# kevin-robb/live_ekf_slam

Measured on AMD Instinct MI355X. Metric: EKF predict-update steps/sec @ L=50, batch=65536; fp64 state RMSE vs ref, higher is better.
Workload: dtype f64

## Files before the change

### live_ekf_slam_amd/csrc/ekf_kernel_impl.h

```cpp
#pragma once
#include "ekf_kernel.h"

#include <stdio.h>

#include <type_traits>

#include "../../include/slam_batch.h"
#include "ekf_model.h"
#include "slam_rng.h"
#include "sim_device.h"

namespace slam {

template <int NMAX, int W, int KG_, int UNR_, int KP_ = 0>
struct EkfGeom {
    static constexpr int TPB = 64 * W;
    static constexpr int LDP = (NMAX + 2) & ~1;
    static constexpr int LMAX = (NMAX - 3) / 2;
    static constexpr int KCAP = LMAX > 0 ? LMAX : 1;
    static constexpr int KG = KG_;
    static constexpr int KP = KP_ > 0 ? KP_ : ((KG_ > 5 && NMAX > 43 && W < 5) ? 3 : (KG_ > 4 ? 4 : KG_));
    static constexpr int KLOOP = 2 * KP;
    static constexpr int TS = 3 + 2 * KP;
    static constexpr int UNR = UNR_;
};

template <int VEC>
constexpr int hp_substride(int ldp) {
    int hs = (ldp + VEC - 1) / VEC;
    while ((hs % 16) != (16 / VEC) && (hs % 16) != 16 - (16 / VEC)) ++hs;
    return hs;
}

#ifdef SLAM_ABLATE
#define SLAM_DBG(x) (x)
#else
#define SLAM_DBG(x) 0
#endif

#ifndef SLAM_SLEEP_RING
#define SLAM_SLEEP_RING 1
#endif
#ifndef SLAM_SLEEP_LEADER
#define SLAM_SLEEP_LEADER 2
#endif
#ifndef SLAM_SLEEP_PASS
#define SLAM_SLEEP_PASS 1
#endif
#ifndef SLAM_PASS_MIN
#define SLAM_PASS_MIN 4
#endif
#ifndef SLAM_W1_WAVES
#define SLAM_W1_WAVES 3
#endif
#ifndef SLAM_SD
#define SLAM_SD 3
#endif
#ifndef SLAM_CTRL_ILP
#define SLAM_CTRL_ILP 1
#endif
#ifndef SLAM_CTRL_SG
#define SLAM_CTRL_SG 3
#endif
#ifndef SLAM_PRIO_THIN
#define SLAM_PRIO_THIN 2
#endif

#define SLAM_STAMP(i)                                                                    \
    do {                                                                                 \
        if (prof_on && tid == 0) {                                                       \
            const unsigned long long now_ = __builtin_readcyclecounter();                \
            p.prof[(size_t)blockIdx.x * kEkfProfSlots + (i)] += now_ - tprev;                            \
            tprev = now_;                                                                \
        }                                                                                \
    } while (0)

typedef double dbl2_t __attribute__((ext_vector_type(2)));
typedef float flt4_t __attribute__((ext_vector_type(4)));
template <class ST> struct Vec16;
template <> struct Vec16<double> {
    static constexpr int VEC = 2;
    typedef dbl2_t type;
};
template <> struct Vec16<float> {
    static constexpr int VEC = 4;
    typedef flt4_t type;
};

__device__ __forceinline__ int opaque(int v) {
    asm volatile("" : "+v"(v));
    return v;
}

typedef const __attribute__((address_space(4))) EkfStepParams* EkfColdParams;
__device__ __forceinline__ EkfColdParams ekf_cold_params() {
    EkfColdParams k = (EkfColdParams)__builtin_amdgcn_kernarg_segment_ptr();
    asm volatile("" : "+s"(k));
    return k;
}
struct EkfSimCold {
    uint64_t seed;
    int64_t inst0;
    double d_max, th_max, range_max, fov_min, fov_max;
};
struct EkfMapCold {
    const double* map;
    const double* map_each;
    const int32_t* L_each;
    int32_t map_stride, L;
};
struct EkfSimNoiseCold {
    double sV00, sV11, sW00, sW11;
    const NoiseRow* noise_each;
    int32_t sim;
};

__device__ __forceinline__ double rdlane(double v, int l) {
    const int lo = __builtin_amdgcn_readlane(__double2loint(v), l);
    const int hi = __builtin_amdgcn_readlane(__double2hiint(v), l);
    return __hiloint2double(hi, lo);
}

__device__ __forceinline__ unsigned hi_abs(double v) {
    return (unsigned)(__double_as_longlong(v) >> 32) & 0x7fffffffu;
}

template <int NMAX, int W, int KG_, int UNR_, class ST, int PIPE, bool MULTI, int KP_ = 0>
__global__ __launch_bounds__(64 * W, (W >= 2 ? 4 : SLAM_W1_WAVES)) void ekf_step_kernel(const EkfStepParams p) {
    using G = EkfGeom<NMAX, W, KG_, UNR_, KP_>;
    constexpr int TPB = G::TPB, LDP = G::LDP, KCAP = G::KCAP, LMAX = G::LMAX, KG = G::KG, KP = G::KP, KLOOP = G::KLOOP, TS = G::TS, UNR = G::UNR;

    __shared__ double s_xt[LDP];
    __shared__ double s_xp[LDP];
    __shared__ double s_R[TS * LDP];
    __shared__ double s_C[TS * LDP];
    __shared__ double2 s_K[KG * LDP];
    constexpr int VEC = Vec16<ST>::VEC;
    constexpr int HS = hp_substride<VEC>(LDP), HPW = (VEC - 1) * HS + (LDP + VEC - 1) / VEC;
    __shared__ double2 s_HP[KG * HPW];
    __shared__ double s_sc[16];
    constexpr int SD = SLAM_SD;
    __shared__ float s_meas[SD * 3 * KCAP];
    __shared__ double s_tru[SD * 6];
    __shared__ int s_kraw[SD];
    __shared__ int s_sim[2];
    __shared__ int s_ids[LMAX > 0 ? LMAX : 1];
    __shared__ int s_didx[2 * KCAP];
    __shared__ int s_next[2 * 4];
    __shared__ double s_ps[2 * 10];
    __shared__ int s_chunk;
    __shared__ int s_T[TS];
    __shared__ signed char s_slot[LDP];
    __shared__ signed char s_need[TS];
    __shared__ int s_misc[8];
    __shared__ double s_keep[4];
    __shared__ int s_kh[8];
    __shared__ int s_ring[8];
    __shared__ int s_pass[4];
    __shared__ int s_wend[KG];
    __shared__ unsigned s_cnt[4];

    const int b = blockIdx.x;
    const int tid = threadIdx.x;
    const int lane = tid & 63;
    const FilterNoise nz = filter_noise(p, b);
    if (p.long_mode == 1) {
        const int kk = p.meas_count_in[b];
        if ((kk < p.k_stride_in ? kk : p.k_stride_in) > p.long_cap) return;
    }

    const bool dump_meas = p.meas_out != nullptr;
    const bool prof_on = (p.dbg & 4) && p.prof != nullptr;
    unsigned long long tprev = prof_on ? __builtin_readcyclecounter() : 0ull;
    if (prof_on && tid < 64) p.prof[(size_t)blockIdx.x * kEkfProfSlots + tid] = 0ull;
    typedef typename Vec16<ST>::type VT;
    constexpr int ESZ = (int)sizeof(ST);
    auto hpi = [](int c) -> int { return (c & (VEC - 1)) * HS + (c / VEC); };
    const int T = MULTI ? p.T : 1;
    ST* const PA = const_cast<ST*>(static_cast<const ST*>(p.P)) + (size_t)b * p.pstride;
    ST* const PB = static_cast<ST*>(p.P_out) + (size_t)b * p.pstride;
    ST* const Pfinal = PA;
    ST* Pcur = PA;
    ST* __restrict__ xb = static_cast<ST*>(p.x) + (size_t)b * p.xstride;
    constexpr bool kWide = sizeof(ST) == 8;
    int flags = p.flags[b];
    const int M_init = p.M[b];
    double xpre[(LDP + TPB - 1) / TPB];
#pragma unroll
    for (int u = 0; u < (LDP + TPB - 1) / TPB; ++u) {
        const int i = tid + TPB * u;
        xpre[u] = (i < p.xstride && i < LDP) ? (double)xb[i] : 0.0;
    }
    const int idpre = (tid < p.L_max) ? p.ids[(size_t)b * p.L_max + tid] : 0;
    double keep0 = 0.0;
    if (p.sim && tid < 64) {
        if (tid < 3) keep0 = p.truth[3 * (size_t)b + tid];
        if (tid == 3) keep0 = p.err_sum[b];
    }
    const int n_init = 3 + 2 * M_init;
    const int ts0 = p.timestep[b];

    if (flags & SLAM_INST_INDEX_OOR) {
        return;
    }

#pragma unroll
    for (int u = 0; u < (LDP + TPB - 1) / TPB; ++u) {
        const int i = tid + TPB * u;
        if (i < LDP) {
            const double v = i < n_init ? xpre[u] : 0.0;
            s_xt[i] = v;
            s_xp[i] = v;
        }
    }
    if (tid < M_init) s_ids[tid] = idpre;
    if (tid < 4) s_keep[tid] = keep0;
#pragma unroll 1
    for (int i = tid; i < LDP; i += TPB) s_slot[i] = (signed char)(i < 3 ? i : -1);
    if (tid < TS) {
        s_T[tid] = tid < 3 ? tid : -1;
        s_need[tid] = (signed char)(tid < 3 ? 1 : 0);
    }
    if (tid < 8) s_kh[tid] = 0;
    if (tid < KG) s_wend[tid] = 0;
    if (tid < 2) s_sim[tid] = 0;
    if (tid < 4) s_cnt[tid] = tid == 1 ? (unsigned)((n_init + M_init / 2 + 8) * ESZ / 8) : 0u;
    auto count_pass = [](unsigned* cnt, int vec16, int nupd) {
        atomicAdd(&cnt[0], (unsigned)vec16);
        atomicAdd(&cnt[2], 1u);
        atomicAdd(&cnt[3], (unsigned)nupd);
    };
    auto count_other = [](unsigned* cnt, int elems) { atomicAdd(&cnt[1], (unsigned)(elems * ESZ) / 8u); };

#include "ekf_step_prestep.h"
#include "ekf_step_control.h"
#include "ekf_step_stream.h"
    if (W == 1) pregather(tid, TPB);
    else if (tid >= 64) pregather(tid - 64, TPB - 64);
    if (tid == TPB - 1) count_other(s_cnt, 6 * n_init);
    if (tid < 64) prestep(0);
    if (tid >= TPB - 3) s_need[tid - (TPB - 3)] = 0;
    SLAM_STAMP(1);

    bool wd_fired = false;
    int frz_at = -1, frz_M = 0, frz_n = 0;
    const ST* frz_P = nullptr;
#pragma unroll 1
    for (int t = 0; t < T; ++t) {
    const ST* const Pin = Pcur;
    const int pb = t & 1;
    const float* const meas_t = s_meas + (t % SD) * 3 * KCAP;
    int* const didx_t = s_didx + pb * KCAP;
    const int M_old = M;
    const int n_old = na;
    if (tid < 8) s_misc[tid] = 0;
    __builtin_amdgcn_s_setprio(SLAM_PRIO_THIN);
    __syncthreads();
    const int kraw = s_next[4 * pb];
    if (kraw > KCAP) flags |= SLAM_INST_CAPACITY;
    const int k = kraw < KCAP ? kraw : KCAP;
    if (tid == 0) s_kh[k < 7 ? k : 7] += 1;
    if (p.sim && dump_meas && t == T - 1) {
        const EkfColdParams pc = ekf_cold_params();
        const int kso = pc->k_stride_out;
        float* const mo = pc->meas_out + (size_t)b * kso * 3;
        for (int i = tid; i < 3 * k && i < 3 * kso; i += TPB) mo[i] = meas_t[i];
        if (tid == 0) pc->meas_count_out[b] = k;
    }
    const int room_ins = (p.L_max < LMAX ? p.L_max : LMAX) - M_old;
    const int n_ins = p.id_known ? s_next[4 * pb + 1] : (k < room_ins ? k : (room_ins > 0 ? room_ins : 0));
    const bool frz_top = p.id_known && s_next[4 * pb + 2];
    if (p.id_known && s_next[4 * pb + 3]) flags |= SLAM_INST_CAPACITY;
    SLAM_STAMP(2);

#include "ekf_step_decoupled.h"
#include "ekf_step_lockstep.h"
    const int te = opaque(tid);
    for (int i = te; i < na; i += TPB) {
        const ST sv = (ST)s_xp[i];
        s_xt[i] = (double)sv;
        s_xp[i] = (double)sv;
        const unsigned h0 = hi_abs((double)sv);
        hiacc = hiacc > h0 ? hiacc : h0;
    }
    if constexpr (!kWide) {
        if (t + 1 < T) {
            const int nTl = s_misc[5];
#pragma unroll 1
            for (int i = te; i < nTl * LDP; i += TPB) {
                s_R[i] = (double)(ST)s_R[i];
                s_C[i] = (double)(ST)s_C[i];
            }
        }
    }
    if (s_misc[6]) flags |= SLAM_INST_S_SINGULAR;
    const bool nonfinite = __syncthreads_or(hiacc >= 0x7ff00000u);
    if (nonfinite) flags |= SLAM_INST_NONFINITE;

    if (na != nf) {
        const int ldf = ekf_ld(nf, ESZ), lda = ekf_ld(na, ESZ);
        if (tid == 0) count_other(s_cnt, 2 * na * na);
#pragma unroll 1
        for (int r = 0; r < na; ++r) {
            ST tmp[(LDP + TPB - 1) / TPB];
#pragma unroll
            for (int u = 0; u < (LDP + TPB - 1) / TPB; ++u) {
                const int c = te + TPB * u;
                tmp[u] = c < na ? Pout[(size_t)r * ldf + c] : (ST)0;
            }
            __syncthreads();
#pragma unroll
            for (int u = 0; u < (LDP + TPB - 1) / TPB; ++u) {
                const int c = te + TPB * u;
                if (c < lda) Pout[(size_t)r * lda + c] = tmp[u];
            }
            __syncthreads();
        }
    }
    if ((p.dbg & 32) && p.prof != nullptr && tid == 0 && t < kEkfProfSlots)
        p.prof[(size_t)blockIdx.x * kEkfProfSlots + t] = (wall_clock64() << 4) | (unsigned long long)(k < 15 ? k : 15);
    Pcur = Pout;
    SLAM_STAMP(10);
    }

    if (wd_fired) {
        finish(0, M, flags | SLAM_INST_WATCHDOG | SLAM_INST_INDEX_OOR, true);
        return;
    }
    if (frz_at >= 0) {
        __syncthreads();
        if (Pfinal != frz_P) {
            const int nn = frz_n * ekf_ld(frz_n, ESZ);
            if (tid == 0) count_other(s_cnt, 2 * nn);
            for (int i = tid; i < nn; i += TPB) Pfinal[i] = frz_P[i];
            __syncthreads();
        }
        finish(frz_at, frz_M, flags | SLAM_INST_INDEX_OOR, true);
        return;
    }
    if (Pcur != Pfinal) {
        __syncthreads();
        const int nn = na * ekf_ld(na, ESZ);
        if (tid == 0) count_other(s_cnt, 2 * nn);
        for (int i = tid; i < nn; i += TPB) Pfinal[i] = Pcur[i];
        __syncthreads();
    }

    finish(T, M, flags, false);
    SLAM_STAMP(8);
}

template <int NMAX, int W, int KG_, int UNR_, class ST, int PIPE, int KP_>
hipError_t launch_variant(const EkfStepParams& p, hipStream_t stream) {
    if (ekf_device_cmds(p) && p.T > 1)
        hipLaunchKernelGGL((ekf_step_kernel<NMAX, W, KG_, UNR_, ST, PIPE, true, KP_>), dim3(p.B), dim3(64 * W), 0, stream, p);
    else
        hipLaunchKernelGGL((ekf_step_kernel<NMAX, W, KG_, UNR_, ST, PIPE, false, KP_>), dim3(p.B), dim3(64 * W), 0, stream, p);
    return hipGetLastError();
}

template <int NMAX, int W, int KG_, int UNR_, class ST, int PIPE, int KP_>
hipError_t variant_info(int multi, EkfKernelInfo* out) {
    const void* fn = multi ? reinterpret_cast<const void*>(&ekf_step_kernel<NMAX, W, KG_, UNR_, ST, PIPE, true, KP_>)
                           : reinterpret_cast<const void*>(&ekf_step_kernel<NMAX, W, KG_, UNR_, ST, PIPE, false, KP_>);
    hipFuncAttributes a;
    hipError_t e = hipFuncGetAttributes(&a, fn);
    if (e != hipSuccess) return e;
    int nb = 0;
    e = hipOccupancyMaxActiveBlocksPerMultiprocessor(&nb, fn, 64 * W, 0);
    if (e != hipSuccess) return e;
    snprintf(out->name, sizeof(out->name), "ekf_step_kernel<%d,%d,%d,%d,%s,%d,%s,%d>", NMAX, W, KG_, UNR_,
             sizeof(ST) == 8 ? "double" : "float", PIPE, multi ? "true" : "false", KP_);
    out->lds_bytes = (int)a.sharedSizeBytes;
    out->vgprs = a.numRegs;
    out->sgprs = 0;
    out->threads = 64 * W;
    out->wg_per_cu = nb;
    return hipSuccess;
}

}
```

### live_ekf_slam_amd/csrc/ekf_step_control.h

```cpp

    auto leader_chain = [&](int ii, int si, float r_m, float b_m, double (&H)[8], double& nu0, double& nu1, double (&Si)[4]) -> bool {
        const double* const xl = p.lm_from_pred ? s_xp : s_xt;
        const double dx = xl[ii] - s_xp[0], dy = xl[ii + 1] - s_xp[1];
        const float dist = (float)sqrt(dx * dx + dy * dy);
        const double dd = (double)dist, d2 = (double)(dist * dist);
        const int hl = lane & 7;
        const bool usey = (hl == 1) || (hl == 3) || (hl == 4) || (hl == 6);
        const bool neg = (hl == 0) || (hl == 1) || (hl == 5) || (hl == 6);
        double num = usey ? dy : dx;
        num = neg ? -num : num;
        const double q = num / (hl < 4 ? dd : d2);
        const float angf = (float)rem2pi(det_atan2(dy, dx) - s_xp[2]);
        const float nu0f = r_m - dist - nz.w_r;
        const float nu1f = b_m - angf - nz.w_b;
        nu0 = (double)nu0f; nu1 = (double)nu1f;
#pragma unroll
        for (int j = 0; j < 8; ++j) H[j] = rdlane(q, j);
        const double h00 = H[0], h01 = H[1], h03 = H[2], h04 = H[3], h10 = H[4], h11 = H[5], h12 = -1.0, h13 = H[6], h14 = H[7];
        const int cs = lane < 3 ? lane : (lane == 3 ? ii : ii + 1);
        const double p0 = s_R[cs], p1 = s_R[LDP + cs], p2 = s_R[2 * LDP + cs], pi = s_R[si * LDP + cs], pj = s_R[(si + 1) * LDP + cs];
        const double gx = ((h00 * p0 + h01 * p1) + h03 * pi) + h04 * pj;
        const double gy = (((h10 * p0 + h11 * p1) + h12 * p2) + h13 * pi) + h14 * pj;
        const double g0x = rdlane(gx, 0), g1x = rdlane(gx, 1), g2x = rdlane(gx, 2), gix = rdlane(gx, 3), gjx = rdlane(gx, 4);
        const double g0y = rdlane(gy, 0), g1y = rdlane(gy, 1), g2y = rdlane(gy, 2), giy = rdlane(gy, 3), gjy = rdlane(gy, 4);
        double S[4];
        S[0] = ((g0x * h00 + g1x * h01) + gix * h03) + gjx * h04;
        S[1] = (((g0x * h10 + g1x * h11) + g2x * h12) + gix * h13) + gjx * h14;
        S[2] = ((g0y * h00 + g1y * h01) + giy * h03) + gjy * h04;
        S[3] = (((g0y * h10 + g1y * h11) + g2y * h12) + giy * h13) + gjy * h14;
        S[0] = S[0] + nz.W00;
        S[3] = S[3] + nz.W11;
        return inv2x2_lu(S, Si);
    };

    auto form_known = [&](const int* didx_g, int k, int l0, int lim, int nsrc, int& l1_out, int& nT_out) -> int {
        const int l1 = (k - l0 < lim) ? k : l0 + lim;
        const int ng = l1 - l0;
        const int idx = (lane < ng) ? didx_g[l0 + lane] : -1;
        const int myii = idx >= 0 ? 3 + 2 * idx : -1;
        const int cur = (lane < KP) ? s_T[3 + 2 * lane] : -1;
        bool dupl = false, has = false, keep = false;
#pragma unroll
        for (int w = 0; w < KP; ++w) {
            const int ii_w = __builtin_amdgcn_readlane(myii, w), cur_w = __builtin_amdgcn_readlane(cur, w);
            dupl = dupl || (w < lane && ii_w == myii);
            has = has || (cur_w >= 0 && cur_w == myii);
            keep = keep || (ii_w >= 0 && ii_w == cur);
        }
        const bool wantv = myii >= 0 && !dupl;
        const bool release = lane < KP && cur >= 0 && !keep;
        if (release) {
            s_slot[cur] = (signed char)-1; s_slot[cur + 1] = (signed char)-1;
            s_T[3 + 2 * lane] = -1; s_T[4 + 2 * lane] = -1;
        }
        const bool freeslot = lane < KP && (cur < 0 || !keep);
        const unsigned long long fmask = __ballot(freeslot);
        const bool needs = wantv && !has;
        const unsigned long long nmask = __ballot(needs);
        const int rank = __popcll(nmask & ((1ull << lane) - 1ull));
        int j = 0;
        {
            unsigned long long fm = fmask;
#pragma unroll
            for (int w = 0; w < KP; ++w) {
                const int lowest = __ffsll((long long)fm) - 1;
                if (w == rank) j = lowest;
                fm &= fm - 1ull;
            }
        }
        bool gath = false;
        if (needs) {
            s_T[3 + 2 * j] = myii; s_T[4 + 2 * j] = myii + 1;
            s_slot[myii] = (signed char)(3 + 2 * j); s_slot[myii + 1] = (signed char)(4 + 2 * j);
            const signed char nd = (signed char)(myii < nsrc ? 1 : 2);
            s_need[3 + 2 * j] = nd; s_need[4 + 2 * j] = nd;
            gath = nd == 1;
        }
        unsigned long long occ = __ballot(lane < KP && cur >= 0 && keep);
        {
            unsigned long long fm = fmask;
            const int ntake = __popcll(nmask);
#pragma unroll
            for (int w = 0; w < KP; ++w) {
                const int lowest = __ffsll((long long)fm) - 1;
                if (w < ntake && lowest >= 0) occ |= 1ull << lowest;
                fm &= fm - 1ull;
            }
        }
        l1_out = l1;
        nT_out = occ ? 5 + 2 * (63 - __clzll((long long)occ)) : 3;
        return __ballot(gath) != 0ull ? 1 : 0;
    };

    auto thin_downdate = [&](int j0, int jstride, int s0, int sstride, int nTd, int nd, const double2* __restrict__ Ku,
                             const double2* __restrict__ HPu) {
        const int* const Ttab = s_T;
#pragma unroll 1
        for (int j = j0; j < nd; j += jstride) {
            const double2 kj = Ku[j], hj = HPu[hpi(j)];
#pragma unroll 2
            for (int sl = s0; sl < nTd; sl += sstride) {
                const int t_s = Ttab[sl];
                if ((unsigned)t_s < (unsigned)nd) {
                    const double2 kt = Ku[t_s], ht = HPu[hpi(t_s)];
                    const int i = sl * LDP + j;
                    s_R[i] = ekf_downdate(s_R[i], kt.x, kt.y, hj.x, hj.y);
                    s_C[i] = ekf_downdate(s_C[i], kj.x, kj.y, ht.x, ht.y);
                }
            }
        }
    };

    constexpr int NU = (LDP + 63) / 64;
    auto thin_downdate_ctl = [&](int nTd, int nd, const double2* __restrict__ Ku, const double2* __restrict__ HPu, const double2 (&kj)[NU],
                                 const double2 (&hj)[NU]) {
        constexpr int SG = SLAM_CTRL_SG;
        int tsv[TS];
#pragma unroll
        for (int sl = 0; sl < TS; ++sl) tsv[sl] = s_T[sl];
#pragma unroll
        for (int s0 = 0; s0 < TS; s0 += SG) {
            if (s0 >= nTd) break;
            double2 kt[SG], ht[SG];
            double rv[SG][NU], cv[SG][NU];
            bool ok[SG];
#pragma unroll
            for (int g = 0; g < SG; ++g) {
                const int sl = s0 + g < TS ? s0 + g : TS - 1;
                const int t_s = tsv[sl];
                ok[g] = s0 + g < nTd && (unsigned)t_s < (unsigned)nd;
                const int tc = ok[g] ? t_s : 0;
                kt[g] = Ku[tc]; ht[g] = HPu[hpi(tc)];
#pragma unroll
                for (int u = 0; u < NU; ++u) {
                    const int j = lane + 64 * u;
                    const int i = sl * LDP + (j < LDP ? j : 0);
                    rv[g][u] = s_R[i]; cv[g][u] = s_C[i];
                }
            }
#pragma unroll
            for (int g = 0; g < SG; ++g) {
                if (!ok[g]) continue;
                const int sl = s0 + g;
#pragma unroll
                for (int u = 0; u < NU; ++u) {
                    const int j = lane + 64 * u;
                    if (j < nd) {
                        const int i = sl * LDP + j;
                        s_R[i] = ekf_downdate(rv[g][u], kt[g].x, kt[g].y, hj[u].x, hj[u].y);
                        s_C[i] = ekf_downdate(cv[g][u], kj[u].x, kj[u].y, ht[g].x, ht[g].y);
                    }
                }
            }
        }
    };
```

### live_ekf_slam_amd/csrc/ekf_step_decoupled.h

```cpp

    if constexpr (MULTI && W >= 2) {
        auto fastable = [&](int tq) -> bool {
            const int* nx = s_next + 4 * (tq & 1);
            constexpr int kStepMax = sizeof(ST) == 8 ? KLOOP : (KLOOP < KG ? KLOOP : KG);
            return nx[0] <= kStepMax && nx[1] == 0 && nx[2] == 0 && nx[3] == 0;
        };
        const bool fast_ok = p.id_known && !dump_meas && fastable(t) &&
                             !SLAM_DBG(p.dbg & (2 | 16 | 64));
        if (fast_ok) {
            const int n = na, ldn = ekf_ld(n, ESZ);
            ST* const Pbuf = Pcur;
            constexpr int kFirstStreamer = 1;
            constexpr int NS = W - kFirstStreamer;
            constexpr bool kGen = W >= 2;
            if (tid == 0) {
                s_ring[0] = nu; s_ring[1] = 0; s_ring[2] = 0; s_ring[3] = 0; s_ring[4] = t; s_ring[5] = 0; s_ring[6] = 0; s_ring[7] = 0;
                s_pass[0] = 0; s_pass[1] = 0; s_pass[2] = 0; s_pass[3] = 0;
            }
            __syncthreads();
            auto ld_i = [](int* q) -> int { return __hip_atomic_load(q, __ATOMIC_RELAXED, __HIP_MEMORY_SCOPE_WORKGROUP); };
            auto st_i = [](int* q, int v) { __hip_atomic_store(q, v, __ATOMIC_RELAXED, __HIP_MEMORY_SCOPE_WORKGROUP); };
            constexpr int kSpinBudget = 1 << 21;
            auto spin_over = [&](int& spins) -> bool {
                spins += 1;
                if (spins > kSpinBudget) st_i(&s_ring[2], 1);
                return ld_i(&s_ring[2]) != 0;
            };

            bool is_streamer = true;
            if (tid < 64) {
                is_streamer = false;
                __builtin_amdgcn_s_setprio(3);
                int tt = t;
                int pub = nu;
                int fl_or = 0;
                bool first_it = true;
#pragma unroll 1
                for (;;) {
                    const int pq = tt & 1;
                    const float* const meas_q = s_meas + (tt % SD) * 3 * KCAP;
                    const int* const didx_q = s_didx + pq * KCAP;
                    const int kq = s_next[4 * pq];
                    if (lane == 0) st_i(&s_sim[1], tt);
                    if (!first_it && lane == 0) s_kh[kq < 7 ? kq : 7] += 1;
                    first_it = false;
                    if (lane < 3) s_xp[lane] = s_ps[10 * pq + lane];
                    SLAM_STAMP(16);
                    int lastu = -1;
                    if constexpr (!kWide) {
                        const bool isupd = lane < kq && didx_q[lane] >= 0;
                        const unsigned long long um = __ballot(isupd);
                        lastu = um ? 63 - __clzll((long long)um) : -1;
                    }
                    int l0q = 0, l1q, nTq;
#pragma unroll 1
                    do {
                    const int needg = form_known(didx_q, kq, l0q, KP, n, l1q, nTq);
                    SLAM_STAMP(17);
                    const bool veh = s_need[0] == 1;
                    if (needg || veh) {
                        if (lane == 0) st_i(&s_ring[6], 1);
                        __builtin_amdgcn_fence(__ATOMIC_SEQ_CST, "workgroup");
                        for (int sp = 0; ld_i(&s_ring[7]) && !spin_over(sp);) __builtin_amdgcn_s_sleep(1);
                        __builtin_amdgcn_fence(__ATOMIC_ACQUIRE, "workgroup");
                        const int app = ld_i(&s_ring[1]);
                        int sl = 0;
#pragma unroll 1
                        while (sl < nTq) {
                            constexpr int GB = 2;
                            int ss[GB], ts[GB], nb = 0;
#pragma unroll
                            for (int g = 0; g < GB; ++g) { ss[g] = 0; ts[g] = 0; }
#pragma unroll 1
                            while (sl < nTq && nb < GB) {
                                if (s_need[sl] == 1) {
#pragma unroll
                                    for (int g = 0; g < GB; ++g)
                                        if (g == nb) { ss[g] = sl; ts[g] = s_T[sl]; }
                                    nb += 1;
                                }
                                sl += 1;
                            }
                            if (nb == 0) break;
                            if (lane == 0) count_other(s_cnt, 2 * nb * n);
#pragma unroll 1
                            for (int j = lane; j < LDP; j += 64) {
                                double rv[GB], cv[GB];
                                const int jc = j < n ? j : 0;
#pragma unroll
                                for (int g = 0; g < GB; ++g) {
                                    rv[g] = (double)Pbuf[(size_t)ts[g] * ldn + jc];
                                    cv[g] = (double)Pbuf[(size_t)jc * ldn + ts[g]];
                                }
#pragma unroll 1
                                for (int u = app; u < pub; ++u) {
                                    const int us = u % KG;
                                    const double2* Ku = s_K + us * LDP;
                                    const double2* HPu = s_HP + us * HPW;
                                    const double2 kj = Ku[jc], hj = HPu[hpi(jc)];
                                    bool we = false;
                                    if constexpr (!kWide) we = s_wend[us] != 0;
#pragma unroll
                                    for (int g = 0; g < GB; ++g) {
                                        const double2 kt = Ku[ts[g]], ht = HPu[hpi(ts[g])];
                                        rv[g] = ekf_downdate(rv[g], kt.x, kt.y, hj.x, hj.y);
                                        cv[g] = ekf_downdate(cv[g], kj.x, kj.y, ht.x, ht.y);
                                        if constexpr (!kWide) {
                                            if (we) { rv[g] = (double)(ST)rv[g]; cv[g] = (double)(ST)cv[g]; }
                                        }
                                    }
                                }
#pragma unroll
                                for (int g = 0; g < GB; ++g)
                                    if (g < nb) {
                                        s_R[ss[g] * LDP + j] = j < n ? rv[g] : 0.0;
                                        s_C[ss[g] * LDP + j] = j < n ? cv[g] : 0.0;
                                    }
                            }
#pragma unroll
                            for (int g = 0; g < GB; ++g)
                                if (g < nb && ss[g] >= 3 && lane < 3) {
                                    s_R[ss[g] * LDP + lane] = s_C[lane * LDP + ts[g]];
                                    s_C[ss[g] * LDP + lane] = s_R[lane * LDP + ts[g]];
                                }
                        }
                        if (lane == 0) st_i(&s_ring[6], 0);
                    }
                    if (lane < TS) s_need[lane] = 0;
                    SLAM_STAMP(18);
                    if (l0q == 0) {
                        const double* const ps = s_ps + 10 * pq;
                        const double* const r2o = s_R + 2 * LDP;
                        const double* const c2o = s_C + 2 * LDP;
                        const double fa = ps[3], fb = ps[4];
                        const double p22 = r2o[2];
                        auto predicted = [&](double tv, int r, int cc) -> double {
                            const double f_r = r == 0 ? fa : fb;
                            if (r < 2) tv = tv + f_r * r2o[cc];
                            if (cc < 2) {
                                double a2 = c2o[r];
                                if (r < 2) a2 = a2 + f_r * p22;
                                tv = tv + a2 * (cc == 0 ? fa : fb);
                            }
                            if (r < 2 && cc < 2) tv = tv + ps[5 + 2 * r + cc];
                            if (r == 2 && cc == 2) tv = tv + nz.V11;
                            return tv;
                        };
                        double n_r0 = 0.0, n_r1 = 0.0, n_c0 = 0.0, n_c1 = 0.0, n_22 = 0.0;
                        const int t_s = (lane >= 2 && lane < nTq) ? s_T[lane] : -1;
                        const bool thin_l = (unsigned)t_s < (unsigned)n;
                        if (thin_l) {
                            n_r0 = predicted(s_R[lane * LDP + 0], t_s, 0);
                            n_r1 = predicted(s_R[lane * LDP + 1], t_s, 1);
                            n_c0 = predicted(s_C[lane * LDP + 0], 0, t_s);
                            n_c1 = predicted(s_C[lane * LDP + 1], 1, t_s);
                            if (lane == 2) n_22 = predicted(p22, 2, 2);
                        }
#pragma unroll
                        for (int u = 0; u < (LDP + 63) / 64; ++u) {
                            const int j = lane + 64 * u;
                            if (j >= 2 && j < n) {
                                const double r2 = r2o[j], c2 = c2o[j];
                                s_R[j] = ekf_pred_row(s_R[j], fa, r2);
                                s_R[LDP + j] = ekf_pred_row(s_R[LDP + j], fb, r2);
                                s_C[j] = ekf_pred_col(s_C[j], c2, fa);
                                s_C[LDP + j] = ekf_pred_col(s_C[LDP + j], c2, fb);
                            }
                        }
                        if (lane < 2) {
                            const int j = lane;
                            const double v00 = predicted(s_R[j], 0, j), v10 = predicted(s_R[LDP + j], 1, j);
                            const double w00 = predicted(s_C[j], j, 0), w10 = predicted(s_C[LDP + j], j, 1);
                            s_R[j] = v00; s_R[LDP + j] = v10; s_C[j] = w00; s_C[LDP + j] = w10;
                        }
                        if (thin_l) {
                            s_R[lane * LDP + 0] = n_r0; s_R[lane * LDP + 1] = n_r1;
                            s_C[lane * LDP + 0] = n_c0; s_C[lane * LDP + 1] = n_c1;
                            if (lane == 2) { s_R[2 * LDP + 2] = n_22; s_C[2 * LDP + 2] = n_22; }
                        }
                    }
                    SLAM_STAMP(19);
#pragma unroll 1
                    for (int l = l0q; l < l1q; ++l) {
                        const int idx = didx_q[l];
                        if (idx < 0) continue;
                        const float r_m = meas_q[3 * l + 1], b_m = meas_q[3 * l + 2];
                        const int ii = 3 + 2 * idx;
                        const int si = s_slot[ii];
                        double H[8], Si[4], nu0, nu1;
                        if (!leader_chain(ii, si, r_m, b_m, H, nu0, nu1, Si)) fl_or |= SLAM_INST_S_SINGULAR;
                        SLAM_STAMP(20);
                        for (int sp = 0; pub - ld_i(&s_ring[1]) >= KG && !spin_over(sp);) __builtin_amdgcn_s_sleep(SLAM_SLEEP_RING);
                        if (ld_i(&s_ring[2])) break;
                        SLAM_STAMP(21);
                        const int slot = pub % KG;
                        double2* __restrict__ HPu = s_HP + slot * HPW;
                        double2* __restrict__ Ku = s_K + slot * LDP;
                        double2 kreg[NU], hreg[NU];
#pragma unroll
                        for (int u = 0; u < NU; ++u) { kreg[u] = make_double2(0.0, 0.0); hreg[u] = make_double2(0.0, 0.0); }
                        if (!SLAM_DBG(p.dbg & 512)) {
                            const double h00 = H[0], h01 = H[1], h03 = H[2], h04 = H[3], h10 = H[4], h11 = H[5], h12 = -1.0, h13 = H[6], h14 = H[7];
                            const double* Ri = s_R + si * LDP;
                            const double* Rj = s_R + (si + 1) * LDP;
                            const double* Ci = s_C + si * LDP;
                            const double* Cj = s_C + (si + 1) * LDP;
#pragma unroll
                            for (int u = 0; u < (LDP + 63) / 64; ++u) {
                                const int c = lane + 64 * u;
                                double2 hp = make_double2(0.0, 0.0), kk = make_double2(0.0, 0.0);
                                if (c < n) {
                                    const double p0 = s_R[c], p1 = s_R[LDP + c], p2 = s_R[2 * LDP + c], pi = Ri[c], pj = Rj[c];
                                    hp.x = ((h00 * p0 + h01 * p1) + h03 * pi) + h04 * pj;
                                    hp.y = (((h10 * p0 + h11 * p1) + h12 * p2) + h13 * pi) + h14 * pj;
                                    const double q0 = s_C[c], q1 = s_C[LDP + c], q2 = s_C[2 * LDP + c], qi = Ci[c], qj = Cj[c];
                                    const double phx = ((q0 * h00 + q1 * h01) + qi * h03) + qj * h04;
                                    const double phy = (((q0 * h10 + q1 * h11) + q2 * h12) + qi * h13) + qj * h14;
                                    kk.x = phx * Si[0] + phy * Si[2];
                                    kk.y = phx * Si[1] + phy * Si[3];
                                    double xv = s_xp[c] + (kk.x * nu0 + kk.y * nu1);
                                    if (c == 2) xv = rem2pi(xv);
                                    s_xp[c] = xv;
                                }
                                if (c < LDP) { HPu[hpi(c)] = hp; Ku[c] = kk; }
                                kreg[u] = kk; hreg[u] = hp;
                            }
                        }
                        if (!kWide && lane == 0) s_wend[slot] = (l == lastu) ? 1 : 0;
                        __builtin_amdgcn_fence(__ATOMIC_RELEASE, "workgroup");
                        pub += 1;
                        if (lane == 0) st_i(&s_ring[0], pub);
                        SLAM_STAMP(22);
                        if (!SLAM_DBG(p.dbg & 256)) {
#if SLAM_CTRL_ILP
                            thin_downdate_ctl(nTq, n, Ku, HPu, kreg, hreg);
#else
                            thin_downdate(lane, 64, 0, 1, nTq, n, Ku, HPu);
#endif
                        }
                    }
                    l0q = l1q;
                    } while (l0q < kq && !ld_i(&s_ring[2]));
                    if (ld_i(&s_ring[2])) break;
                    SLAM_STAMP(23);
                    if (p.sim && lane == 0) {
                        const double* tru = s_tru + (tt % SD) * 6 + 3;
                        const double ex = (double)(float)s_xp[0] - tru[0], ey = (double)(float)s_xp[1] - tru[1];
                        s_keep[3] = s_keep[3] + sqrt(ex * ex + ey * ey);
                    }
#pragma unroll 1
                    for (int i = lane; i < n; i += 64) {
                        const ST sv = (ST)s_xp[i];
                        s_xt[i] = (double)sv;
                        s_xp[i] = (double)sv;
                        const unsigned h0 = hi_abs((double)sv);
                        hiacc = hiacc > h0 ? hiacc : h0;
                    }
                    if constexpr (!kWide) {
                        const int nel = nTq * LDP;
#pragma unroll 1
                        for (int i0 = lane; i0 < nel; i0 += 256) {
                            double rv[4], cv[4];
#pragma unroll
                            for (int u = 0; u < 4; ++u) {
                                const int i = i0 + 64 * u < nel ? i0 + 64 * u : i0;
                                rv[u] = s_R[i]; cv[u] = s_C[i];
                            }
#pragma unroll
                            for (int u = 0; u < 4; ++u) {
                                const int i = i0 + 64 * u;
                                if (i < nel) { s_R[i] = (double)(ST)rv[u]; s_C[i] = (double)(ST)cv[u]; }
                            }
                        }
                    }
                    if ((p.dbg & 32) && p.prof != nullptr && lane == 0 && tt < kEkfProfSlots)
                        p.prof[(size_t)blockIdx.x * kEkfProfSlots + tt] = (wall_clock64() << 4) | (unsigned long long)(kq < 15 ? kq : 15);
                    tt += 1;
                    SLAM_STAMP(24);
                    if (tt >= T) break;
                    if constexpr (kGen) {
                        for (int sp = 0; ld_i(&s_sim[0]) <= tt && !spin_over(sp);) __builtin_amdgcn_s_sleep(1);
                        __builtin_amdgcn_fence(__ATOMIC_ACQUIRE, "workgroup");
                    }
                    SLAM_STAMP(26);
                    prestep(tt);
                    SLAM_STAMP(25);
                    if (!fastable(tt)) break;
                }
                if (lane == 0) {
                    s_ring[4] = tt;
                    s_ring[5] = fl_or;
                    __builtin_amdgcn_fence(__ATOMIC_RELEASE, "workgroup");
                    st_i(&s_ring[3], 1);
                    if (ld_i(&s_ring[2])) st_i(&s_ring[6], 0);
                }
                __builtin_amdgcn_s_setprio(0);
            }
            if (is_streamer) {
                __builtin_amdgcn_s_setprio(0);
                const bool leader = (tid >> 6) == kFirstStreamer;
#ifdef SLAM_PASS_MIN_FORCE
                constexpr int kPassMinCfg = SLAM_PASS_MIN_FORCE;
#else
#ifdef SLAM_PASS_MIN_F32
                constexpr int kPassMinF32 = SLAM_PASS_MIN_F32;
#else
                constexpr int kPassMinF32 = KG > 4 ? KG - 2 : 3;
#endif
                constexpr int kPassMinCfg = kWide ? (KG > SLAM_PASS_MIN + 1 ? KG - 1 : SLAM_PASS_MIN) : kPassMinF32;
#endif
                constexpr int kPassMin = kPassMinCfg < KG ? kPassMinCfg : KG;
                int seen = 0;
                int sp = 0;
#pragma unroll 1
                for (;;) {
                    if (leader) {
                        int app, pend;
                        bool stop = false;
#pragma unroll 1
                        for (;;) {
                            if (spin_over(sp)) { stop = true; break; }
                            app = ld_i(&s_ring[1]);
                            pend = ld_i(&s_ring[0]) - app;
                            const int ex = ld_i(&s_ring[3]);
                            if (pend > 0 && (pend >= kPassMin || ex) && !ld_i(&s_ring[6])) break;
                            if (ex && pend == 0) {
                                if (ld_i(&s_ring[0]) - app == 0) { stop = true; break; }
                                continue;
                            }
                            if constexpr (W == 2) {
                                const int ts = ld_i(&s_sim[0]);
                                if (ts < T && ts < ld_i(&s_sim[1]) + SD && !ex) {
                                    simgen(ts);
                                    __builtin_amdgcn_fence(__ATOMIC_RELEASE, "workgroup");
                                    if (lane == 0) st_i(&s_sim[0], ts + 1);
                                    continue;
                                }
                            }
                            __builtin_amdgcn_s_sleep(SLAM_SLEEP_LEADER);
                        }
                        int cnt = pend < KG ? pend : KG;
                        if constexpr (!kWide) {
                            if (!stop) {
                                while (cnt > 0 && !ld_i(&s_wend[(app + cnt - 1) % KG])) cnt -= 1;
                                if (cnt == 0) { __builtin_amdgcn_s_sleep(1); continue; }
                            }
                        }
                        if (!stop) {
                            if (lane == 0) st_i(&s_ring[7], 1);
                            __builtin_amdgcn_fence(__ATOMIC_SEQ_CST, "workgroup");
                            if (ld_i(&s_ring[6])) {
                                if (lane == 0) st_i(&s_ring[7], 0);
                                __builtin_amdgcn_s_sleep(1);
                                continue;
                            }
                        }
                        if (lane == 0) {
                            s_pass[1] = app;
                            s_pass[2] = stop ? -1 : cnt;
                            s_pass[3] = 0;
                            s_chunk = 0;
                            if (!stop) count_pass(s_cnt, 2 * n * (ldn / VEC), cnt);
                            __builtin_amdgcn_fence(__ATOMIC_RELEASE, "workgroup");
                            st_i(&s_pass[0], seen + 1);
                        }
                    }
                    while (ld_i(&s_pass[0]) <= seen && !spin_over(sp)) {
                        if constexpr (kGen && W >= 3) {
                            if ((tid >> 6) == W - 1) {
                                const int ts = ld_i(&s_sim[0]);
                                if (ts < T && ts < ld_i(&s_sim[1]) + SD && !ld_i(&s_ring[3])) {
                                    simgen(ts);
                                    __builtin_amdgcn_fence(__ATOMIC_RELEASE, "workgroup");
                                    if (lane == 0) st_i(&s_sim[0], ts + 1);
                                    continue;
                                }
                            }
                        }
                        __builtin_amdgcn_s_sleep(SLAM_SLEEP_PASS);
                    }
                    seen += 1;
                    sp = 0;
                    __builtin_amdgcn_fence(__ATOMIC_ACQUIRE, "workgroup");
                    const int lo = ld_i(&s_pass[1]), cnt = ld_i(&s_pass[2]);
                    if (cnt < 0 || ld_i(&s_ring[2])) break;
                    PassArgs pa;
                    pa.src = Pbuf; pa.dst = Pbuf; pa.mid = nullptr;
                    pa.nf = n; pa.ldd = ldn; pa.lds = ldn; pa.nsrc = n; pa.nu = cnt; pa.lo = lo;
                    stream_pass(std::integral_constant<int, 2>{}, pa);
                    __builtin_amdgcn_fence(__ATOMIC_RELEASE, "workgroup");
                    if (lane == 0) atomicAdd(&s_pass[3], 1);
                    if (leader) {
                        while (ld_i(&s_pass[3]) < NS && !spin_over(sp)) __builtin_amdgcn_s_sleep(1);
                        sp = 0;
                        if (lane == 0) {
                            if (!(p.dbg & 128)) st_i(&s_ring[1], lo + cnt);
                            st_i(&s_ring[7], 0);
                        }
                    }
                }
            }
            __syncthreads();
            if (s_ring[2]) {
                wd_fired = true;
                break;
            }
            nu = 0;
            flags |= s_ring[5];
            const int t_next = s_ring[4];
            write_vehicle(Pbuf, n);
            if (tid < KG) s_wend[tid] = 0;
            if (__syncthreads_or(hiacc >= 0x7ff00000u)) flags |= SLAM_INST_NONFINITE;
            t = t_next - 1;
            continue;
        }
    }
```

Before: 72.05 million.

## Defer ring wait past thin downdate and source tracked K/HP from registers

```diff
diff --git a/live_ekf_slam_amd/csrc/ekf_kernel_impl.h b/live_ekf_slam_amd/csrc/ekf_kernel_impl.h
--- a/live_ekf_slam_amd/csrc/ekf_kernel_impl.h
+++ b/live_ekf_slam_amd/csrc/ekf_kernel_impl.h
@@ -55,9 +55,6 @@
 #endif
 #ifndef SLAM_SD
 #define SLAM_SD 3
-#endif
-#ifndef SLAM_CTRL_ILP
-#define SLAM_CTRL_ILP 1
 #endif
 #ifndef SLAM_CTRL_SG
 #define SLAM_CTRL_SG 3
@@ -158,6 +155,7 @@
     __shared__ int s_ring[8];
     __shared__ int s_pass[4];
     __shared__ int s_wend[KG];
+    __shared__ double2 s_tKH[2 * (TS - 3)];
     __shared__ unsigned s_cnt[4];
 
     const int b = blockIdx.x;
diff --git a/live_ekf_slam_amd/csrc/ekf_step_control.h b/live_ekf_slam_amd/csrc/ekf_step_control.h
--- a/live_ekf_slam_amd/csrc/ekf_step_control.h
+++ b/live_ekf_slam_amd/csrc/ekf_step_control.h
@@ -112,8 +112,7 @@
     };
 
     constexpr int NU = (LDP + 63) / 64;
-    auto thin_downdate_ctl = [&](int nTd, int nd, const double2* __restrict__ Ku, const double2* __restrict__ HPu, const double2 (&kj)[NU],
-                                 const double2 (&hj)[NU]) {
+    auto thin_downdate_ctl = [&](int nTd, int nd, const double2 (&kj)[NU], const double2 (&hj)[NU]) {
         constexpr int SG = SLAM_CTRL_SG;
         int tsv[TS];
 #pragma unroll
@@ -129,8 +128,12 @@
                 const int sl = s0 + g < TS ? s0 + g : TS - 1;
                 const int t_s = tsv[sl];
                 ok[g] = s0 + g < nTd && (unsigned)t_s < (unsigned)nd;
-                const int tc = ok[g] ? t_s : 0;
-                kt[g] = Ku[tc]; ht[g] = HPu[hpi(tc)];
+                if (sl < 3) {
+                    kt[g] = make_double2(rdlane(kj[0].x, sl), rdlane(kj[0].y, sl));
+                    ht[g] = make_double2(rdlane(hj[0].x, sl), rdlane(hj[0].y, sl));
+                } else {
+                    kt[g] = s_tKH[2 * (sl - 3)]; ht[g] = s_tKH[2 * (sl - 3) + 1];
+                }
 #pragma unroll
                 for (int u = 0; u < NU; ++u) {
                     const int j = lane + 64 * u;
diff --git a/live_ekf_slam_amd/csrc/ekf_step_decoupled.h b/live_ekf_slam_amd/csrc/ekf_step_decoupled.h
--- a/live_ekf_slam_amd/csrc/ekf_step_decoupled.h
+++ b/live_ekf_slam_amd/csrc/ekf_step_decoupled.h
@@ -190,9 +190,8 @@
                         double H[8], Si[4], nu0, nu1;
                         if (!leader_chain(ii, si, r_m, b_m, H, nu0, nu1, Si)) fl_or |= SLAM_INST_S_SINGULAR;
                         SLAM_STAMP(20);
-                        for (int sp = 0; pub - ld_i(&s_ring[1]) >= KG && !spin_over(sp);) __builtin_amdgcn_s_sleep(SLAM_SLEEP_RING);
+                        const bool direct = pub - ld_i(&s_ring[1]) < KG;
                         if (ld_i(&s_ring[2])) break;
-                        SLAM_STAMP(21);
                         const int slot = pub % KG;
                         double2* __restrict__ HPu = s_HP + slot * HPW;
                         double2* __restrict__ Ku = s_K + slot * LDP;
@@ -210,6 +209,7 @@
                                 const int c = lane + 64 * u;
                                 double2 hp = make_double2(0.0, 0.0), kk = make_double2(0.0, 0.0);
                                 if (c < n) {
+                                    const int sc = s_slot[c];
                                     const double p0 = s_R[c], p1 = s_R[LDP + c], p2 = s_R[2 * LDP + c], pi = Ri[c], pj = Rj[c];
                                     hp.x = ((h00 * p0 + h01 * p1) + h03 * pi) + h04 * pj;
                                     hp.y = (((h10 * p0 + h11 * p1) + h12 * p2) + h13 * pi) + h14 * pj;
@@ -221,22 +221,34 @@
                                     double xv = s_xp[c] + (kk.x * nu0 + kk.y * nu1);
                                     if (c == 2) xv = rem2pi(xv);
                                     s_xp[c] = xv;
-                                }
-                                if (c < LDP) { HPu[hpi(c)] = hp; Ku[c] = kk; }
+                                    if (sc >= 3) { s_tKH[2 * (sc - 3)] = kk; s_tKH[2 * (sc - 3) + 1] = hp; }
+                                }
+                                if (direct && c < LDP) { HPu[hpi(c)] = hp; Ku[c] = kk; }
                                 kreg[u] = kk; hreg[u] = hp;
                             }
                         }
-                        if (!kWide && lane == 0) s_wend[slot] = (l == lastu) ? 1 : 0;
-                        __builtin_amdgcn_fence(__ATOMIC_RELEASE, "workgroup");
-                        pub += 1;
-                        if (lane == 0) st_i(&s_ring[0], pub);
+                        auto publish = [&]() {
+                            if (!kWide && lane == 0) s_wend[slot] = (l == lastu) ? 1 : 0;
+                            __builtin_amdgcn_fence(__ATOMIC_RELEASE, "workgroup");
+                            pub += 1;
+                            if (lane == 0) st_i(&s_ring[0], pub);
+                        };
+                        if (direct) publish();
                         SLAM_STAMP(22);
-                        if (!SLAM_DBG(p.dbg & 256)) {
-#if SLAM_CTRL_ILP
-                            thin_downdate_ctl(nTq, n, Ku, HPu, kreg, hreg);
-#else
-                            thin_downdate(lane, 64, 0, 1, nTq, n, Ku, HPu);
-#endif
+                        if (!SLAM_DBG(p.dbg & 256))
+                            thin_downdate_ctl(nTq, n, kreg, hreg);
+                        SLAM_STAMP(23);
+                        if (!direct) {
+                            for (int sp = 0; pub - ld_i(&s_ring[1]) >= KG && !spin_over(sp);) __builtin_amdgcn_s_sleep(SLAM_SLEEP_RING);
+                            if (ld_i(&s_ring[2])) break;
+                            SLAM_STAMP(21);
+#pragma unroll
+                            for (int u = 0; u < (LDP + 63) / 64; ++u) {
+                                const int c = lane + 64 * u;
+                                if (c < LDP) { HPu[hpi(c)] = hreg[u]; Ku[c] = kreg[u]; }
+                            }
+                            publish();
+                            SLAM_STAMP(27);
                         }
                     }
                     l0q = l1q;
```

After: 71.49 million. Within noise of the previous version (-0.8%).
